# vLAR-group/unMORE

Hardware: AMD Instinct MI355X
Metric: images/sec (train fwd+bwd) ObjectnessNet ViT-B/16 384x384 (higher is better)
Workload: dtype bf16

## Files before the change

### include/umr.h

```cpp
#ifndef UMR_H
#define UMR_H
#include <stdint.h>

#ifdef __cplusplus
extern "C" {
#endif

typedef void* umr_stream_t;

enum umr_status { UMR_OK = 0, UMR_ERR_INVALID = -1, UMR_ERR_UNSUPPORTED = -2, UMR_ERR_HIP = -1000 };
enum umr_dtype { UMR_F32 = 0, UMR_BF16 = 1, UMR_BF16X3 = 2 };

int umr_version(void);
const char* umr_last_error_string(void);

enum umr_f32_mode { UMR_F32_EXACT = 0, UMR_F32_X3 = 1, UMR_F32_X3_FAST = 2 };
int umr_set_f32_mode(int mode);
int umr_get_f32_mode(void);

int umr_set_cu_budget(int cus);
int umr_get_cu_budget(void);

int umr_set_debug_option(const char* name, const char* value);
int umr_get_debug_option(const char* name, int* value, int* is_set);
// ... 40 lines not shown
int umr_unsplit3(const void* src, float* dst, int64_t rows, int K, int64_t ld_src, int64_t ld_dst, umr_stream_t stream);
int umr_split3_rows(const float* src, void* dst, int64_t rows, int K, int64_t ld_src, int64_t ld_dst, int rows_in, int rows_out,
                    int row_off, umr_stream_t stream);
int umr_gemm_nt_rowreduce_ok(const umr_gemm_desc* d);

typedef struct umr_gemm_tn_desc {
    const void* dY;
    const void* X;
    float* dW;
    float* dbias;
    void* workspace;
    int64_t workspace_bytes;
    int64_t lddy, ldx, lddw;
    int32_t M, N, K;
    int32_t dtype;
    int32_t accumulate;
    int32_t conv, nb, H, W, Cin, Ho, Wo;
    int32_t dy_rows_in, dy_rows_out, dy_row_off;
    int32_t x_rows_in, x_rows_out, x_row_off;
} umr_gemm_tn_desc;

int64_t umr_gemm_tn_workspace(const umr_gemm_tn_desc* d);
int umr_gemm_tn(const umr_gemm_tn_desc* d, umr_stream_t stream);

int umr_layernorm_fwd(const void* x, const float* gamma, const float* beta, void* y, float* mean, float* rstd,
                      int M, int D, float eps, int dtype, umr_stream_t stream);
int64_t umr_layernorm_bwd_workspace(int M, int D);
int umr_layernorm_bwd(const void* dy, const void* x, const float* gamma, const float* mean, const float* rstd,
                      const void* dres, void* dx, float* dgamma, float* dbeta, int accumulate, void* workspace,
                      int64_t workspace_bytes, int M, int D, int dtype, umr_stream_t stream);
int umr_layernorm_bwd_rows(const void* dy, const void* x, const float* gamma, const float* mean, const float* rstd,
                           const void* dres, void* dx, void* workspace, int64_t workspace_bytes, int M, int D, int dtype,
                           umr_stream_t stream);
int umr_layernorm_bwd_params(const void* workspace, int64_t workspace_bytes, float* dgamma, float* dbeta, int accumulate,
                             int M, int D, umr_stream_t stream);

int64_t umr_attention_bwd_workspace(int B, int N, int heads);
int umr_attention_fwd(const void* qkv, void* out, float* lse, int B, int N, int heads, int head_dim, int dtype,
                      umr_stream_t stream);
int umr_attention_bwd(const void* qkv, const void* out, const void* dout, const float* lse, float* dsum_ws, void* dqkv,
                      int B, int N, int heads, int head_dim, int dtype, umr_stream_t stream);

int umr_patchify(const float* images, void* out, int B, int H, int W, int patch, int ldk, int dtype, umr_stream_t stream);
int umr_bilinear_fwd(const void* x, void* y, int B, int Hi, int Wi, int Ho, int Wo, int C, int align_corners, int dtype, umr_stream_t stream);
int umr_bilinear_bwd(const void* dy, void* dx, int B, int Hi, int Wi, int Ho, int Wo, int C, int align_corners, int dtype, umr_stream_t stream);
#define UMR_BILINEAR_RELU 1
// ... 189 lines not shown
```

### unmore_amd/_lib.py

```python
import ctypes
import os
import subprocess

_HERE = os.path.dirname(os.path.abspath(__file__))
LIB_PATH = os.environ.get("UMR_LIB") or os.path.join(_HERE, "lib", "libumr.so")
CSRC = os.path.join(_HERE, "csrc")

F32, BF16, BF16X3 = 0, 1, 2
EPI_BIAS, EPI_ADD_AUX, EPI_MASK_RELU, EPI_MASK_DGELU, EPI_ADD_AUX2, EPI_OUT_F32, EPI_ROWBIAS, EPI_OUT_X3 = 1, 2, 4, 8, 16, 32, 64, 128
EPI_AUX_X3, EPI_AUX2_X3, EPI_C2_X3 = 256, 512, 1024
ACT_NONE, ACT_RELU, ACT_GELU, ACT_TANH = 0, 1, 2, 3
ACT_SIGMOID = 5
F32_EXACT, F32_X3, F32_X3_FAST = 0, 1, 2

_vp, _i32, _i64 = ctypes.c_void_p, ctypes.c_int32, ctypes.c_int64


class GemmDesc(ctypes.Structure):
    _fields_ = [("A", _vp), ("B", _vp), ("C", _vp), ("C2", _vp), ("bias", _vp), ("aux", _vp),
                ("aux2", _vp), ("rowbias", _vp),
                ("lda", _i64), ("ldb", _i64), ("ldc", _i64), ("ldc2", _i64), ("ldaux", _i64), ("ldaux2", _i64),
                ("M", _i32), ("N", _i32), ("K", _i32), ("dtype", _i32),
                ("flags", _i32), ("act", _i32), ("c2_mode", _i32), ("rows_per_batch", _i32),
                ("conv", _i32), ("nb", _i32), ("H", _i32), ("W", _i32), ("Cin", _i32), ("Ho", _i32), ("Wo", _i32),
                ("a_rows_in", _i32), ("a_rows_out", _i32), ("a_row_off", _i32),
                ("c_rows_in", _i32), ("c_rows_out", _i32), ("c_row_off", _i32), ("aux_mod", _i32),
                ("red_w", _vp), ("red_out", _vp), ("red_c", _i32), ("no_store", _i32)]


class GemmTnDesc(ctypes.Structure):
    _fields_ = [("dY", _vp), ("X", _vp), ("dW", _vp), ("dbias", _vp), ("workspace", _vp),
                ("workspace_bytes", _i64), ("lddy", _i64), ("ldx", _i64), ("lddw", _i64),
                ("M", _i32), ("N", _i32), ("K", _i32), ("dtype", _i32), ("accumulate", _i32),
                ("conv", _i32), ("nb", _i32), ("H", _i32), ("W", _i32), ("Cin", _i32), ("Ho", _i32), ("Wo", _i32),
                ("dy_rows_in", _i32), ("dy_rows_out", _i32), ("dy_row_off", _i32),
                ("x_rows_in", _i32), ("x_rows_out", _i32), ("x_row_off", _i32)]


class AdamPackEntry(ctypes.Structure):
    _fields_ = [("p", _vp), ("g", _vp), ("m", _vp), ("v", _vp), ("dst_lin", _vp), ("dst_t", _vp), ("n", _i64), ("N", _i32), ("K", _i32),
                ("blk_start", _i64)]


class BnBwdDesc(ctypes.Structure):
    _fields_ = [("dy", _vp), ("dpool", _vp), ("y", _vp), ("z", _vp * 2), ("mean", _vp * 2), ("rstd", _vp * 2), ("gamma", _vp * 2),
                ("dgamma", _vp * 2), ("dbeta", _vp * 2), ("dz", _vp * 2), ("g_out", _vp), ("workspace", _vp), ("workspace_bytes", _i64),
                ("rows_per_batch", _i64), ("pool_scale", ctypes.c_float), ("M", _i32), ("C", _i32), ("nbranch", _i32), ("dtype", _i32)]


class RaggedSrc(ctypes.Structure):
    _fields_ = [("f32", _vp), ("u8", _vp), ("H", _i32), ("W", _i32)]


class CpPair(ctypes.Structure):
    _fields_ = [("l_image", _vp), ("l_masks", _vp), ("l_boxes", _vp), ("u_image", _vp), ("u_masks", _vp), ("out_image", _vp), ("out_masks", _vp),
                ("word_off", _i64), ("inter_off", _i64), ("row_off", _i64), ("choice_off", _i64),
                ("Hl", _i32), ("Wl", _i32), ("Nl", _i32), ("Hu", _i32), ("Wu", _i32), ("Nu", _i32), ("nc", _i32), ("h_new", _i32), ("w_new", _i32),
                ("h_shift", _i32), ("w_shift", _i32), ("rh", ctypes.c_float), ("rw", ctypes.c_float), ("sx", ctypes.c_float), ("sy", ctypes.c_float),
                ("reserved", _i32)]
# ... 27 lines not shown
    "umr_label_synthesis_workspace": [_i32, _i32, _i32],
    "umr_label_synthesis": [_vp, _vp, _vp, _vp, _vp, _vp, _i64, _i32, _i32, _i32, _i32, _vp],
    "umr_label_synthesis_cropped": [_vp, _vp, _vp, _vp, _vp, _vp, _vp, _i64, _i32, _i32, _i32, _i32, _vp],
    "umr_crop_resize_batch": [_vp, _vp, _vp, _i32, _i32, _i32, _i32, _i32, _i32, _i32, _vp],
    "umr_distance_transform_workspace": [_i32, _i32, _i32],
    "umr_distance_transform": [_vp, _vp, _vp, _i64, _i32, _i32, _i32, _i32, _vp],
    "umr_bg_square_workspace": [_i32, _i64],
    "umr_bg_square": [_vp, _vp, _vp, _i64, _i32, _i32, _i64, _vp],
    "umr_crop_resize_ragged": [_vp, _vp, _vp, _vp, _vp, _i32, _i32, _i32, _i32, _vp],
    "umr_im2col_nchw": [_vp, _vp, _i32, _i32, _i32, _i32, _i32, _i32, _i32, _i32, _i32, _i32, _vp],
    "umr_maxpool3x3s2": [_vp, _vp, _i32, _i32, _i32, _i32, _i32, _vp],
    "umr_bn_fold": [_vp, _vp, _vp, _vp, _vp, _f32, _vp, _vp, _i32, _i32, _i32, _i32, _vp],
    "umr_bn_train_workspace": [_i32, _i32],
    "umr_bn_train_stats": [_vp, _vp, _vp, _vp, _vp, _vp, _vp, _i64, _i32, _i32, _f32, _f32, _i32, _vp],
    "umr_bn_train_apply": [_vp, _vp, _vp, _vp, _vp, _vp, _vp, _vp, _vp, _vp, _vp, _vp, _i32, _i32, _i32, _i32, _vp],
    "umr_bn_train_bwd_reduce": [_vp, _vp],
    "umr_bn_train_bwd_apply": [_vp, _vp],
    "umr_maxpool3x3s2_bwd": [_vp, _vp, _vp, _i32, _i32, _i32, _i32, _i32, _vp],
    "umr_stuff2_add": [_vp, _vp, _i32, _i32, _i32, _i32, _i32, _vp],
    "umr_bce_sigmoid": [_vp, _vp, _vp, _vp, _i32, _vp],
    "umr_head_out_finish": [_vp, _i32, _vp, _vp, _i64, _i32, _i32, _i32, _vp],
    "umr_gemm_tn": [_vp, _vp],
    "umr_gemm_tn_workspace": [_vp],
    "umr_layernorm_fwd": [_vp, _vp, _vp, _vp, _vp, _vp, _i32, _i32, _f32, _i32, _vp],
    "umr_layernorm_bwd_workspace": [_i32, _i32],
    "umr_layernorm_bwd": [_vp, _vp, _vp, _vp, _vp, _vp, _vp, _vp, _vp, _i32, _vp, _i64, _i32, _i32, _i32, _vp],
    "umr_layernorm_bwd_rows": [_vp, _vp, _vp, _vp, _vp, _vp, _vp, _vp, _i64, _i32, _i32, _i32, _vp],
    "umr_layernorm_bwd_params": [_vp, _i64, _vp, _vp, _i32, _i32, _i32, _vp],
    "umr_attention_fwd": [_vp, _vp, _vp, _i32, _i32, _i32, _i32, _i32, _vp],
    "umr_attention_bwd": [_vp, _vp, _vp, _vp, _vp, _vp, _i32, _i32, _i32, _i32, _i32, _vp],
    "umr_attention_bwd_workspace": [_i32, _i32, _i32],
    "umr_patchify": [_vp, _vp, _i32, _i32, _i32, _i32, _i32, _i32, _vp],
    "umr_bilinear_fwd": [_vp, _vp, _i32, _i32, _i32, _i32, _i32, _i32, _i32, _i32, _vp],
    "umr_bilinear_bwd": [_vp, _vp, _i32, _i32, _i32, _i32, _i32, _i32, _i32, _i32, _vp],
    "umr_bilinear_fwd_ex": [_vp, _i64, _vp, _i64, _i32, _i32, _i32, _i32, _i32, _i32, _i32, _i32, _i32, _vp],
    "umr_bilinear_bwd_ex": [_vp, _i64, _vp, _i64, _i32, _i32, _i32, _i32, _i32, _i32, _i32, _i32, _vp],
    "umr_pixel_shuffle": [_vp, _vp, _i32, _i32, _i32, _i32, _i32, _i32, _i32, _vp],
    "umr_zero_stuff2": [_vp, _vp, _i32, _i32, _i32, _i32, _i32, _i32, _i32, _vp],
    "umr_permute4": [_vp, _vp, _vp, _vp, _i64, _i32, _i32, _i32, _vp],
    "umr_segsum": [_vp, _vp, _i32, _i32, _i64, _i64, _i32, _i32, _i32, _i32, _vp],
    "umr_fill_cls": [_vp, _vp, _vp, _i32, _i64, _i32, _i32, _vp],
    "umr_cast": [_vp, _vp, _i64, _f32, _i32, _i32, _vp],
    "umr_scale_by_device_scalar": [_vp, _vp, _vp, _i64, _vp],
    "umr_head_out_fwd": [_vp, _vp, _vp, _vp, _i64, _i32, _i32, _i32, _i32, _i32, _vp],
    "umr_head_out_bwd_workspace": [_i64, _i32],
    "umr_head_out_bwd": [_vp, _vp, _vp, _vp, _vp, _vp, _vp, _vp, _i64, _i64, _i32, _i32, _i32, _i32, _i32, _i32, _vp],
# ... 86 lines not shown
```

### unmore_amd/csrc/gemm_tn.hip

```cpp
#include "umr_common.h"
#include <type_traits>
#include <stdlib.h>

namespace {

constexpr int TN_BN = 128, TN_BK = 128;
constexpr int TN_LDS = 65536;

template <typename T> struct TnTr;
template <> struct TnTr<bf16_t> { static constexpr int ROWS = 64, ROWB = 256, RPI = 4; };
template <> struct TnTr<float> { static constexpr int ROWS = 32, ROWB = 512, RPI = 2; };

__device__ __forceinline__ int tn_swz(int r) { return ((r & 3) << 2) | ((r >> 2) & 3); }

__device__ __forceinline__ void tn_split3(const float (&x)[8], bf16x8& h, bf16x8& m, bf16x8& l) {
#pragma unroll
    for (int e = 0; e < 8; ++e) {
        const bf16_t hh = (bf16_t)x[e];
        const float r = x[e] - (float)hh;
        const bf16_t mm = (bf16_t)r;
        h[e] = hh; m[e] = mm; l[e] = (bf16_t)(r - (float)mm);
    }
}

template <typename T, int CONV, bool X3 = false>
__global__ __launch_bounds__(256, 2) void gemm_tn_kernel(const umr_gemm_tn_desc p, int tiles_k, int rows_per_split,
                                                         float* slab, float* bslab) {
    extern __shared__ __attribute__((aligned(16))) char smem[];
    constexpr int ROWS = TnTr<T>::ROWS, ROWB = TnTr<T>::ROWB, RPI = TnTr<T>::RPI;
    constexpr int EPC = 16 / sizeof(T);
    constexpr int TILE = ROWS * ROWB;
    constexpr int STAGE = 2 * TILE;
    constexpr int CPR = ROWB / 16;
    const int tid = threadIdx.x, lane = tid & 63;
    const int w = __builtin_amdgcn_readfirstlane(tid >> 6);
    const int tile = blockIdx.x, split = blockIdx.y;
    const int tn = tile / tiles_k, tk = tile - tn * tiles_k;
    const int n0 = tn * TN_BN, k0 = tk * TN_BK;
    const int m_begin = split * rows_per_split;
    const int m_end = min(p.M, m_begin + rows_per_split);
    const bool do_bias = (p.dbias != nullptr) && (tk == 0);

    constexpr unsigned OOB = 0x80000000u;
    constexpr int SZ = (int)sizeof(T);
    const int lrow = lane / CPR, lchk = lane % CPR;
    const int stride = (CONV == 2) ? 2 : 1;
    int rr[4], gch[4], k_tap[4], k_ci[4], tky[4], tkx[4];
    unsigned y_vo[4], x_vo[4];
    bool k_ok[4];
#pragma unroll
    for (int i = 0; i < 4; ++i) {
        const int r = (w * 4 + i) * RPI + lrow;
        rr[i] = r;
        gch[i] = (sizeof(T) == 2) ? (lchk ^ tn_swz(r)) : lchk;
        const bool n_ok = (n0 + gch[i] * EPC) < p.N;
        y_vo[i] = n_ok ? (unsigned)(((int64_t)r * p.lddy) * SZ + gch[i] * 16) : OOB;
        const int kc = k0 + gch[i] * EPC;
        k_ok[i] = kc < p.K;
        k_tap[i] = 0;
// ... 250 lines not shown
                }
            }
        }
    }

    float* out = slab + (int64_t)split * p.N * p.K;
#pragma unroll
    for (int nt = 0; nt < 4; ++nt) {
        const int n = n0 + wn * 64 + nt * 16 + li;
        if (n >= p.N) continue;
#pragma unroll
        for (int kt = 0; kt < 4; ++kt) {
            const int k = k0 + wk * 64 + kt * 16 + g * 4;
            if (k >= p.K) continue;
            float* o = out + (int64_t)n * p.K + k;
            if (k + 3 < p.K && (p.K & 3) == 0) *(f32x4*)o = acc[nt][kt];
            else { for (int e = 0; e < 4; ++e) if (k + e < p.K) o[e] = acc[nt][kt][e]; }
        }
        if (do_bias && wk == 0 && g == 0) bslab[(int64_t)split * p.N + n] = accb[nt][0];
    }
}

template <int VEC>
__global__ void tn_reduce_kernel(const float* __restrict__ slab, float* __restrict__ dW, int64_t lddw, int N, int K,
                                 int splits, int accumulate, const float* __restrict__ bslab, float* __restrict__ dbias, int bias_parts) {
    const int64_t total = (int64_t)N * K;
    const int64_t nvec = total / VEC;
    for (int64_t iv = (int64_t)blockIdx.x * blockDim.x + threadIdx.x; iv < nvec; iv += (int64_t)gridDim.x * blockDim.x) {
        const int64_t i = iv * VEC;
        const int n = (int)(i / K), k = (int)(i - (int64_t)n * K);
        float* o = dW + (int64_t)n * lddw + k;
        if (VEC == 4) {
            f32x4 s0 = {0.f, 0.f, 0.f, 0.f}, s1 = s0, s2 = s0, s3 = s0;
            const float* q = slab + i;
            int sp = 0;
            for (; sp + 4 <= splits; sp += 4) {
                s0 += *(const f32x4*)(q + (int64_t)(sp + 0) * total);
                s1 += *(const f32x4*)(q + (int64_t)(sp + 1) * total);
                s2 += *(const f32x4*)(q + (int64_t)(sp + 2) * total);
                s3 += *(const f32x4*)(q + (int64_t)(sp + 3) * total);
            }
            for (; sp < splits; ++sp) s0 += *(const f32x4*)(q + (int64_t)sp * total);
            f32x4 r = (s0 + s1) + (s2 + s3);
            if (accumulate) r += *(const f32x4*)o;
            *(f32x4*)o = r;
        } else {
            float sacc = 0.f;
            for (int sp = 0; sp < splits; ++sp) sacc += slab[(int64_t)sp * total + i];
            *o = accumulate ? (*o + sacc) : sacc;
        }
    }
    if (dbias != nullptr) {
        for (int n = blockIdx.x * blockDim.x + threadIdx.x; n < N; n += gridDim.x * blockDim.x) {
            float b0 = 0.f, b1 = 0.f, b2 = 0.f, b3 = 0.f;
            int sp = 0;
            for (; sp + 4 <= bias_parts; sp += 4) {
                b0 += bslab[(int64_t)(sp + 0) * N + n];
                b1 += bslab[(int64_t)(sp + 1) * N + n];
                b2 += bslab[(int64_t)(sp + 2) * N + n];
                b3 += bslab[(int64_t)(sp + 3) * N + n];
            }
            for (; sp < bias_parts; ++sp) b0 += bslab[(int64_t)sp * N + n];
            const float sacc = (b0 + b1) + (b2 + b3);
            dbias[n] = accumulate ? (dbias[n] + sacc) : sacc;
        }
    }
}

struct TnPlan { int tiles_n, tiles_k, splits, rows_per_split; int64_t ws; bool big; };

}
bool umr_tn256_eligible(const umr_gemm_tn_desc* d, bool force);
void umr_tn256_plan(const umr_gemm_tn_desc* d, int* splits, int* rows_per_split);
int umr_launch_gemm_tn256(const umr_gemm_tn_desc* d, int splits, int rows_per_split, float* slab, float* bslab, hipStream_t s);
namespace {

static int tn_tile_override() {
    return umr_opt_or(UMR_OPT_GEMM_TILE, 0);
}

TnPlan tn_plan(const umr_gemm_tn_desc* d) {
    TnPlan pl;
    pl.big = tn_tile_override() != 128 && umr_tn256_eligible(d, tn_tile_override() == 256);
    if (pl.big) {
        pl.tiles_n = (d->N + 255) / 256;
        pl.tiles_k = (d->K + 255) / 256;
        umr_tn256_plan(d, &pl.splits, &pl.rows_per_split);
        pl.ws = ((int64_t)pl.splits * d->N * d->K + (int64_t)pl.splits * pl.tiles_k * d->N) * 4;
        return pl;
// ... 6 lines not shown
    int64_t max_by_rows = ((int64_t)d->M + rows * 8 - 1) / (rows * 8);
    if (d->M <= 4096) {
        want = (256 + tiles / 2) / tiles;
        max_by_rows = ((int64_t)d->M + rows * 4 - 1) / (rows * 4);
    }
    if (want > max_by_rows) want = max_by_rows;
    if (want < 1) want = 1;
    if (want > 4096) want = 4096;
    int64_t rps = ((int64_t)d->M + want - 1) / want;
    rps = (rps + rows - 1) / rows * rows;
    pl.rows_per_split = (int)rps;
    pl.splits = (int)(((int64_t)d->M + rps - 1) / rps);
    pl.ws = ((int64_t)pl.splits * d->N * d->K + (int64_t)pl.splits * d->N) * 4;
    return pl;
}

}

extern "C" int64_t umr_gemm_tn_workspace(const umr_gemm_tn_desc* d) {
    if (!d || d->M <= 0 || d->N <= 0 || d->K <= 0) return 0;
    return tn_plan(d).ws;
}

extern "C" int umr_gemm_tn(const umr_gemm_tn_desc* d, umr_stream_t stream) {
    UMR_CHECK_ARG(d != nullptr, "gemm_tn: null descriptor");
    UMR_CHECK_ARG(d->dY && d->X && d->dW && d->workspace, "gemm_tn: null operand");
    UMR_CHECK_ARG(d->M > 0 && d->N > 0 && d->K > 0, "gemm_tn: empty problem");
    UMR_CHECK_ARG(d->dtype == UMR_F32 || d->dtype == UMR_BF16 || d->dtype == UMR_BF16X3, "gemm_tn: dtype");
    const int epc = d->dtype == UMR_F32 ? 4 : 8;
    if (d->dtype == UMR_BF16X3) {
        if (d->dy_rows_in > 0 || d->x_rows_in > 0 || d->conv == 2)
            return umr_set_error(UMR_ERR_UNSUPPORTED, "gemm_tn (BF16X3): no row remaps, no stride-2 conv");
        UMR_CHECK_ARG(d->lddy >= 3 * (int64_t)d->N && (d->conv != 0 || d->ldx >= 3 * (int64_t)d->K), "gemm_tn (BF16X3): rows hold three planes (lddy >= 3N, ldx >= 3K)");
    }
    UMR_CHECK_ARG(d->N % epc == 0 && d->lddy % epc == 0, "gemm_tn: N/lddy must be multiples of 16 bytes");
    UMR_CHECK_ARG(d->conv >= 0 && d->conv <= 2, "gemm_tn: conv mode");
    if (d->conv == 0) {
        UMR_CHECK_ARG(d->K % epc == 0 && d->ldx % epc == 0, "gemm_tn: K/ldx must be multiples of 16 bytes");
    } else {
        UMR_CHECK_ARG(d->Cin % epc == 0 && d->K == 9 * d->Cin, "gemm_tn: conv needs Cin % 16B == 0 and K == 9*Cin");
        UMR_CHECK_ARG((int64_t)d->nb * d->Ho * d->Wo == d->M, "gemm_tn: conv M != nb*Ho*Wo");
        const int s = d->conv == 2 ? 2 : 1;
        UMR_CHECK_ARG(d->Ho == (d->H - 1) / s + 1 && d->Wo == (d->W - 1) / s + 1, "gemm_tn: conv output size");
    }
    {
        const int rows = d->dtype == UMR_F32 ? 32 : 64;
        const int64_t sz = d->dtype == UMR_F32 ? 4 : 2;
        const bool remap = d->dy_rows_in > 0 || (d->conv == 0 && d->x_rows_in > 0);
        const bool conv_general = d->conv != 0 && !(d->conv == 1 && d->Wo % rows == 0);
        (void)conv_general;
        if (remap) {
            const int64_t ymax = d->dy_rows_in > 0 ? ((int64_t)d->M / d->dy_rows_in + 1) * d->dy_rows_out : d->M;
            const int64_t xmax = d->x_rows_in > 0 ? ((int64_t)d->M / d->x_rows_in + 1) * d->x_rows_out : d->M;
            if (ymax * d->lddy * sz >= (1ll << 31) || (d->conv == 0 && xmax * d->ldx * sz >= (1ll << 31)))
                return umr_set_error(UMR_ERR_UNSUPPORTED, "gemm_tn: row-remapped operands must be < 2 GiB");
        }
    }
    const TnPlan pl = tn_plan(d);
    UMR_CHECK_ARG(d->workspace_bytes >= pl.ws, "gemm_tn: workspace too small");
    hipStream_t s = (hipStream_t)stream;
    float* slab = (float*)d->workspace;
    float* bslab = slab + (int64_t)pl.splits * d->N * d->K;
    const bool direct = !pl.big && pl.splits == 1 && !d->accumulate && d->lddw == d->K &&
                        ((uintptr_t)d->dW & 15) == 0;
    if (direct) { slab = d->dW; bslab = d->dbias; }
    if (pl.big) {
        const int st = umr_launch_gemm_tn256(d, pl.splits, pl.rows_per_split, slab, bslab, s);
        if (st != UMR_OK) return st;
    } else {
    dim3 g((unsigned)(pl.tiles_n * pl.tiles_k), (unsigned)pl.splits), b(256);
#define LAUNCH(T, CV) hipLaunchKernelGGL((gemm_tn_kernel<T, CV>), g, b, TN_LDS, s, *d, pl.tiles_k, pl.rows_per_split, slab, bslab)
#define LAUNCH_X3(CV) hipLaunchKernelGGL((gemm_tn_kernel<float, CV, true>), g, b, TN_LDS, s, *d, pl.tiles_k, pl.rows_per_split, slab, bslab)
    const int f32_x3 = umr_f32_mode_now() != UMR_F32_EXACT;
    if (d->dtype == UMR_BF16) {
        if (d->conv == 0) LAUNCH(bf16_t, 0); else if (d->conv == 1) LAUNCH(bf16_t, 1); else LAUNCH(bf16_t, 2);
    } else if (f32_x3) {
        if (d->conv == 0) LAUNCH_X3(0); else if (d->conv == 1) LAUNCH_X3(1); else LAUNCH_X3(2);
    } else {
        if (d->conv == 0) LAUNCH(float, 0); else if (d->conv == 1) LAUNCH(float, 1); else LAUNCH(float, 2);
    }
#undef LAUNCH_X3
#undef LAUNCH
    UMR_LAUNCH_CHECK();
    }
    if (direct) return UMR_OK;
    const int64_t total = (int64_t)d->N * d->K;
    const bool v4 = (d->K % 4 == 0) && (d->lddw % 4 == 0) && (((uintptr_t)d->dW & 15) == 0);
    int rb = (int)((total / (v4 ? 4 : 1) + 255) / 256);
    if (rb > 8192) rb = 8192;
    if (rb < 1) rb = 1;
    if (v4)
        hipLaunchKernelGGL(tn_reduce_kernel<4>, dim3(rb), dim3(256), 0, s, slab, d->dW, d->lddw, d->N, d->K, pl.splits,
                           d->accumulate, bslab, d->dbias, pl.big ? pl.splits * pl.tiles_k : pl.splits);
    else
        hipLaunchKernelGGL(tn_reduce_kernel<1>, dim3(rb), dim3(256), 0, s, slab, d->dW, d->lddw, d->N, d->K, pl.splits,
                           d->accumulate, bslab, d->dbias, pl.big ? pl.splits * pl.tiles_k : pl.splits);
    UMR_LAUNCH_CHECK();
    return UMR_OK;
}
```

### unmore_amd/csrc/gemm_tn256.hip

```cpp
#include "umr_common.h"
#include <type_traits>
#include <stdlib.h>

namespace {

constexpr int TSUB = 64 * 256;
constexpr int TBUF = 4 * TSUB;
constexpr int TLDS = 2 * TBUF;

__device__ __forceinline__ int tn_swz2(int r) { return ((r & 3) << 2) | ((r >> 2) & 3); }

template <int CONV, bool PH2, int WF, bool X3 = false>
__global__ __launch_bounds__(512, 2) void gemm_tn256_kernel(const umr_gemm_tn_desc p, int tiles_k, int ntiles, int rows_per_split,
                                                            float* slab, float* bslab, int mapmode, int npairs_arg = 1) {
    extern __shared__ __attribute__((aligned(16))) char smem[];
    constexpr int SZ = 2;
    const int npairs = X3 ? npairs_arg : 1;
    const int xpix = X3 ? 3 * p.Cin : p.Cin;
    constexpr unsigned OOB = 0x80000000u;
    const int tid = threadIdx.x, lane = tid & 63;
    const int w = __builtin_amdgcn_readfirstlane(tid >> 6);
    int bid = blockIdx.x;
    {
        const int nwg = gridDim.x, xcd = bid & 7, q_ = nwg >> 3, r_ = nwg & 7;
// ... 293 lines not shown
        for (int kt = 0; kt < 4; ++kt) {
            const int k = (mapmode & 1) ? k0 + (kt >> 1) * 128 + wk * 32 + (kt & 1) * 16 + g * 4 : k0 + wk * 64 + kt * 16 + g * 4;
            if (k >= p.K) continue;
            float* o = out + (int64_t)n * p.K + k;
            if (k + 3 < p.K && (p.K & 3) == 0) *(f32x4*)o = acc[nt][kt];
            else { for (int e = 0; e < 4; ++e) if (k + e < p.K) o[e] = acc[nt][kt][e]; }
        }
        if (do_bias && wk == 0) {
            float s_ = bsum[nt];
            s_ += __shfl_xor(s_, 16, 64);
            s_ += __shfl_xor(s_, 32, 64);
            if (g == 0) bslab[((int64_t)split * tiles_k + tk) * p.N + n] = s_;
        }
    }
}

}

bool umr_tn256_eligible(const umr_gemm_tn_desc* d, bool force) {
    if (d->dtype != UMR_BF16 && d->dtype != UMR_BF16X3) return false;
    if (d->dy_rows_in > 0 || d->x_rows_in > 0) return false;
    if (d->conv == 2) return false;
    if (d->dtype == UMR_BF16X3) return true;
    if (d->conv == 1 && d->Wo < 64) return false;
    if (force) return true;
    if (d->N < 192 || d->K < 192) return false;
    const int64_t tiles = (int64_t)((d->N + 255) / 256) * ((d->K + 255) / 256);
    return (int64_t)d->M >= 256 * 64 * 16 / (tiles < 1 ? 1 : tiles) && d->M >= 64 * 64;
}

void umr_tn256_plan(const umr_gemm_tn_desc* d, int* splits, int* rows_per_split) {
    const int64_t tiles = (int64_t)((d->N + 255) / 256) * ((d->K + 255) / 256);
    const int x3 = d->dtype == UMR_BF16X3 ? 6 : 1;
    int64_t rounds = (int64_t)d->M * tiles * x3 / (256ll * 4096);
    if (rounds < 1) rounds = 1;
    if (rounds > 4) rounds = 4;
    int64_t want = rounds * 256 / tiles;
    if (want < 1) want = 1;
    const int64_t min_stages = x3 == 6 ? 2 : 16;
    const int64_t max_by_rows = ((int64_t)d->M + 64 * min_stages - 1) / (64 * min_stages);
    if (want > max_by_rows) want = max_by_rows;
    int64_t rps = ((int64_t)d->M + want - 1) / want;
    rps = (rps + 63) / 64 * 64;
    {
        const int64_t cpix = (int64_t)d->Cin * (d->dtype == UMR_BF16X3 ? 3 : 1);
        const int64_t rowb = 2 * (int64_t)(d->conv ? (cpix > d->lddy ? cpix : d->lddy) : (d->ldx > d->lddy ? d->ldx : d->lddy));
        const int64_t halo = d->conv ? (2 * (int64_t)d->W + 4) * cpix * 2 : 0;
        int64_t cap = ((1ll << 31) - halo - 65536) / rowb / 64 * 64;
// ... 6 lines not shown

int umr_launch_gemm_tn256(const umr_gemm_tn_desc* d, int splits, int rows_per_split, float* slab, float* bslab, hipStream_t s) {
    const int tiles_n = (d->N + 255) / 256, tiles_k = (d->K + 255) / 256;
    dim3 g((unsigned)(tiles_n * tiles_k * splits)), b(512);
    constexpr int mapmode = 3;
#define LT(CV, WFV)                                                                                                    \
    do {                                                                                                               \
        UMR_SET_MAX_LDS_ONCE((gemm_tn256_kernel<CV, true, WFV>), TLDS);                                                \
        hipLaunchKernelGGL((gemm_tn256_kernel<CV, true, WFV>), g, b, TLDS, s, *d, tiles_k, tiles_n * tiles_k, rows_per_split, slab, bslab, mapmode, 1); \
    } while (0)
#define LTX(CV, WFV)                                                                                                   \
    do {                                                                                                               \
        UMR_SET_MAX_LDS_ONCE((gemm_tn256_kernel<CV, true, WFV, true>), TLDS);                                          \
        hipLaunchKernelGGL((gemm_tn256_kernel<CV, true, WFV, true>), g, b, TLDS, s, *d, tiles_k, tiles_n * tiles_k, rows_per_split, slab, bslab, mapmode, npairs); \
    } while (0)
    if (d->dtype == UMR_BF16X3) {
        const int npairs = umr_f32_mode_now() == UMR_F32_X3_FAST ? 3 : 6;
        if (d->conv == 0) LTX(0, 0);
        else if (d->Wo % 64 == 0) LTX(1, 1);
        else if (d->Wo >= 64) LTX(1, 0);
        else LTX(1, 2);
    } else if (d->conv == 0) LT(0, 0);
    else if (d->Wo % 64 == 0) LT(1, 1);
    else LT(1, 0);
#undef LTX
#undef LT
    UMR_LAUNCH_CHECK();
    return UMR_OK;
}
```

### unmore_amd/engine.py

```python
import os

import torch

from . import _lib as L
from . import graphs
from . import ops
from .engine_x3 import X3Numerics, _drop_f, _f
from .packs import (ParamGroup, PackCache, _ACT, _pack_conv3, _pack_conv3_dgrad, _pack_convT, _pack_convT_dgrad, _pack_linear,
                    _pack_linear_t, _rep_bias, _unpack_conv3_grad)

CONFIGS = {
    "dpt_large": dict(D=1024, depth=24, heads=16, patch=16, pos_grid=24, hooks=[5, 11, 17, 23], features=[256, 512, 1024, 1024]),
    "dpt_base": dict(D=768, depth=12, heads=12, patch=16, pos_grid=24, hooks=[2, 5, 8, 11], features=[96, 192, 384, 768]),
    "dpt_small": dict(D=384, depth=12, heads=6, patch=16, pos_grid=24, hooks=[2, 5, 8, 11], features=[48, 96, 192, 384]),
    "dpt_large14": dict(D=1024, depth=24, heads=16, patch=14, pos_grid=37, hooks=[5, 11, 17, 23], features=[256, 512, 1024, 1024]),
    "dpt_tiny": dict(D=128, depth=4, heads=2, patch=16, pos_grid=24, hooks=[0, 1, 2, 3], features=[32, 64, 128, 128]),
}

_FUSE_HEAD_OUT = True
_COMMUTE_RESIZE = True


_WGRAD_STREAM = os.environ.get("UMR_WGRAD_STREAM", "auto")
_side_streams = {}


class WgradStream:

    def __init__(self, dev, on):
        self.on = bool(on)
        self.staged = graphs.staged() if self.on else None
        if self.on and self.staged is None:
            self.main = torch.cuda.current_stream(dev)
            key = (dev.index, self.main.cuda_stream)
            if key not in _side_streams:
                if len(_side_streams) > 16:
                    _side_streams.clear()
                _side_streams[key] = torch.cuda.Stream(device=dev)
            self.side = _side_streams[key]

    def run(self, fn, *used):
        if not self.on:
            return fn()
        if self.staged is not None:
            return self.staged.defer(fn, used)
        self.side.wait_stream(self.main)
        graphs.note_fork(self.main, self.side)
# ... 18 lines not shown
        if _WGRAD_STREAM in ("0", "1"):
            return _WGRAD_STREAM == "1"
        return pixels <= graphs.AUTO_MAX_PIXELS


class PlainNumerics:

    def __init__(self, e, P):
        self.e, self.P = e, P

    def val(self, t):
        return t

    def to_dt(self, t):
        return t if self.e.dt == torch.float32 else ops.cast(t, self.e.dt)

    def mm(self, A, wname, kind, bias=None, *, conv=0, act=L.ACT_NONE, want="f", mask=None, dgelu=None, aux=None, aux2=None,
           rowbias=None, rows_per_batch=0, c2_mode=0, c2_want="f", out=None, c_remap=None, aux_mod=0):
        a_t = mask if mask is not None else (dgelu if dgelu is not None else aux)
        return ops.gemm_nt(A, self.e._w(self.P, wname, kind), bias, out=out, aux=a_t, aux2=aux2, rowbias=rowbias,
                           rows_per_batch=rows_per_batch, act=act, mask_relu=mask is not None, mask_dgelu=dgelu is not None,
                           c2_mode=c2_mode, conv=conv, c_remap=c_remap, aux_mod=aux_mod)

    def wgrad(self, dY, X, dW, dbias=None, *, conv=0, wg=None, then=None):
        def launch():
            r = ops.gemm_tn(dY, X, dW=dW, dbias=dbias, conv=conv)
            if then is not None:
                then(r)
            return r
        return launch() if wg is None else wg.run(launch, dY, X)

    def layernorm(self, x, gamma, beta):
        return ops.layernorm_fwd(x, gamma, beta)

    def readout(self, tok, wname, bias, save, B, g, Nt, D):
        P, dt = self.P, self.e.dt
        w_full = self.e.cache.get((wname, "lin", dt), P[wname], lambda: _pack_linear(P[wname], dt))
        rb = ops.gemm_nt(tok, w_full[:, D:], bias, M=B, lda=Nt * D, out_f32=True)
        if save:
            r, rpre = ops.gemm_nt(tok, w_full[:, :D], None, rowbias=rb, rows_per_batch=g, act=L.ACT_GELU, c2_mode=2, M=B * g,
                                  a_remap=(g, Nt, 1))
        else:
            r, rpre = ops.gemm_nt(tok, w_full[:, :D], None, rowbias=rb, rows_per_batch=g, act=L.ACT_GELU, M=B * g,
                                  a_remap=(g, Nt, 1)), None
        return dict(r=r, rpre=rpre)

    def readout_wgrad(self, d_rpre, rs, tok, dW, B, g, Nt):
        ops.gemm_tn(d_rpre, tok, dW=dW, x_remap=(g, Nt, 1), M=B * g)

    def hook_grad(self, d_rpre, sB, wname, dx, B, g, Nt, D):
        dt = self.e.dt
        w = self.P[wname].detach()
# ... 483 lines not shown
                              aux=(hs["h1"] if relu else None), mask_relu=relu)
            del dh2
            hs["h1"] = None
            ops.bilinear_bwd(dh1.view(B, H, W, c1), ph, pw, True, out=dlow[:, c0:c0 + c1].unflatten(0, (nb, ph, pw)))
            del dh1
            wgrad_lin(f"{name}.{idx[0]}.weight", dlow[:, c0:c0 + c1], pl, f"{name}.{idx[0]}.bias")
            bcat[:, c0:c0 + c1].copy_(self._w(P, f"{name}.{idx[0]}.weight", "lin_t"))
            c0 += c1
        dpath = ops.gemm_nt(dlow, bcat, None).view(nb, ph, pw, C)
        S["path"] = None
        S["feat"] = None
        return dpath

    def backward(self, P, S, d_center, d_sdf, G, stage_cb=None, join_at_stages=False):
        cfg = self.cfg
        nx = S["numerics"](self, P)
        mm, val = nx.mm, nx.val
        B, H, W, gh, gw = S["B"], S["H"], S["W"], S["gh"], S["gw"]
        D, heads, p = cfg["D"], cfg["heads"], cfg["patch"]
        g, Nt = gh * gw, gh * gw + 1
        dev = d_center.device
        wg = WgradStream(dev, WgradStream.wanted(B * H * W))
        ln_via = wg.run if wg.staged is not None else None

        def cb(name):
            if join_at_stages:
                wg.join()
            if stage_cb is not None:
                stage_cb(name, wg)
            wg.stage_end()

        def wgrad_lin(name, dy, x, bias_name=None):
            nx.wgrad(dy, x, G[name].view(G[name].shape[0], -1), (G[bias_name] if bias_name else None), wg=wg)

        def wgrad_c3(name, dy, x_nhwc, bias_name=None, conv=1):
            co = G[name].shape[0]
            nx.wgrad(dy.view(-1, co), x_nhwc, None, (G[bias_name] if bias_name else None), conv=conv, wg=wg,
                     then=lambda dwp: _unpack_conv3_grad(dwp, G[name]))

        dpath = nx.heads_backward(S, d_center, d_sdf, G, wgrad_lin, wgrad_c3, lambda: cb("heads"))

        sc = "backbone.scratch."
        d_rn = {}
        for k in (1, 2, 3, 4):
            r_ = sc + f"refinenet{k}."
            fs = S["fus"][k]
            hh, ww = fs["in_hw"]
            nb, Hp, Wp = dpath.shape[0], dpath.shape[1], dpath.shape[2]
            shp = (nb, hh, ww, 256)
            if "u" in fs:
                dul = val(ops.bilinear_bwd(_f(dpath), hh, ww, True)).view(nb * hh * ww, 256)
                wgrad_lin(r_ + "out_conv.weight", dul, fs["u"].view(nb * hh * ww, 256), r_ + "out_conv.bias")
                du = mm(dul, r_ + "out_conv.weight", "lin_t", None).view(*shp)
                del dul
            else:
                dp2 = dpath.view(nb * Hp * Wp, 256)
                wgrad_lin(r_ + "out_conv.weight", dp2, fs["up"].view(nb * Hp * Wp, 256), r_ + "out_conv.bias")
                dup = _f(mm(dp2, r_ + "out_conv.weight", "lin_t", None))
                du = val(ops.bilinear_bwd(dup.view(nb, Hp, Wp, 256), hh, ww, True))
                del dup
            wgrad_c3(r_ + "resConfUnit2.conv2.weight", du, fs["t2"], r_ + "resConfUnit2.conv2.bias")
# ... 118 lines not shown
```

### unmore_amd/ops.py

```python
import collections
import ctypes

import torch

from . import _lib as L
from . import graphs

_DT = {torch.float32: L.F32, torch.bfloat16: L.BF16}


_cur_dev = torch._C._cuda_getDevice
_raw_stream = torch._C._cuda_getCurrentRawStream


def _stream_id(device_index=None):
    return _raw_stream(_cur_dev() if device_index is None else device_index)


def _stream():
    return ctypes.c_void_p(_raw_stream(_cur_dev()))


def _p(t):
    return ctypes.c_void_p(t.data_ptr()) if t is not None else None
# ... 296 lines not shown
        d.aux, d.ldaux = _p(t2), ld
        keep.append(t2)
    if aux2 is not None:
        t2, ld, pl = _x3_operand(aux2, N)
        flags |= L.EPI_ADD_AUX2 | (L.EPI_AUX2_X3 if pl else 0)
        d.aux2, d.ldaux2 = _p(t2), ld
        keep.append(t2)
    if c2_mode:
        assert red_w is None and c_remap is None
        out2 = torch.empty((M_, 3 * N if c2_planes else N), dtype=torch.bfloat16 if c2_planes else torch.float32, device=Ap.device)
        flags |= L.EPI_C2_X3 if c2_planes else 0
        d.C2, d.ldc2, d.c2_mode = _p(out2), out2.stride(0), c2_mode
    d.aux_mod = aux_mod
    d.A, d.B, d.C, d.bias = _p(Ap), _p(Bp), _p(out), _p(bias)
    d.ldb = Bp.stride(0)
    d.M, d.N, d.K, d.dtype = M_, N, K, L.BF16X3
    d.flags, d.act, d.conv = flags, act, conv
    L.check(_timed_call(d), "umr_gemm_nt")
    if red_w is not None:
        return partials
    return (out, out2) if c2_mode else out


def gemm_tn(dY, X, *, dW=None, dbias=None, accumulate=False, conv=0, M=None, dy_remap=None, x_remap=None, lddy=None, ldx=None, x3=False):
    _need_gpu(dY, X)
    dt = L.BF16X3 if x3 else _DT[X.dtype]
    assert dY.dtype == X.dtype and (not x3 or X.dtype == torch.bfloat16)
    pl = 3 if x3 else 1
    d = L.GemmTnDesc()
    dY2 = dY.reshape(-1, dY.shape[-1]) if dY.is_contiguous() else dY
    N = dY2.shape[-1] // pl
    M = dY2.shape[0] if M is None else M
    if conv:
        nb, H, W, Cin = X.shape
        Cin //= pl
        assert X.is_contiguous()
        s = 2 if conv == 2 else 1
        Ho, Wo = (H - 1) // s + 1, (W - 1) // s + 1
        assert M == nb * Ho * Wo
        K = 9 * Cin
        d.nb, d.H, d.W, d.Cin, d.Ho, d.Wo = nb, H, W, Cin, Ho, Wo
        d.ldx = Cin * pl
    else:
        X2 = X.reshape(-1, X.shape[-1]) if X.is_contiguous() else X
        K = X2.shape[-1] // pl
        d.ldx = X2.stride(0) if ldx is None else ldx
    if dW is None:
        dW = torch.empty((N, K), dtype=torch.float32, device=X.device)
        assert not accumulate
    assert dW.dtype == torch.float32 and dW.stride(-1) == 1
    if dbias is not None:
        assert dbias.dtype == torch.float32 and dbias.numel() == N
    d.dY, d.X, d.dW, d.dbias = _p(dY2), _p(X), _p(dW), _p(dbias)
    d.lddy, d.lddw = (dY2.stride(0) if lddy is None else lddy), (dW.stride(0) if dW.dim() == 2 else K)
    if dy_remap is not None:
        d.dy_rows_in, d.dy_rows_out, d.dy_row_off = dy_remap
    if x_remap is not None:
        d.x_rows_in, d.x_rows_out, d.x_row_off = x_remap
    d.M, d.N, d.K, d.dtype, d.accumulate, d.conv = M, N, K, dt, int(accumulate), conv
    need = L.lib().umr_gemm_tn_workspace(ctypes.byref(d))
    ws = _workspace(need, X.device)
    d.workspace, d.workspace_bytes = _p(ws), ws.numel()
    L.check(L.lib().umr_gemm_tn(ctypes.byref(d), _stream()), "umr_gemm_tn")
    return dW


def layernorm_fwd(x, gamma, beta, eps=1e-6, planes=False):
    _need_gpu(x)
    D = x.shape[-1]
    x2 = x.reshape(-1, D)
    M = x2.shape[0]
    mean = torch.empty(M, dtype=torch.float32, device=x.device)
    rstd = torch.empty(M, dtype=torch.float32, device=x.device)
    if planes:
        assert x.dtype == torch.float32
        y = torch.empty((M, 3 * D), dtype=torch.bfloat16, device=x.device)
        L.check(L.lib().umr_layernorm_fwd(_p(x2), _p(gamma), _p(beta), _p(y), _p(mean), _p(rstd), M, D, eps, L.BF16X3, _stream()),
                "umr_layernorm_fwd")
        return y, mean, rstd
    y = torch.empty_like(x2)
    L.check(L.lib().umr_layernorm_fwd(_p(x2), _p(gamma), _p(beta), _p(y), _p(mean), _p(rstd), M, D, eps, _DT[x.dtype], _stream()),
            "umr_layernorm_fwd")
    return y.view(x.shape), mean, rstd


def layernorm_bwd(dy, x, gamma, mean, rstd, dgamma, dbeta, dres=None, accumulate=False, params_via=None):
# ... 553 lines not shown
```

Measured before the change: 356.7.

## Defer and batch split-K weight-gradient reductions across head wgrads

Adds a deferred mode to the TN wgrad GEMM. The split-K slab reduction is recorded instead of launched, and the recorded reductions are run together in one batched kernel at each stage boundary in the heads backward, cutting kernel-launch count. The wgrad kernel grid is also flattened to 1D with an XCD-aware block remap, and the 256-tile path is now taken under force even for small-Wo conv. The cost is a separate workspace allocation per deferred GEMM instead of the shared one, so more memory is held.

```diff
diff --git a/include/umr.h b/include/umr.h
--- a/include/umr.h
+++ b/include/umr.h
@@ -86,6 +86,16 @@
 
 int64_t umr_gemm_tn_workspace(const umr_gemm_tn_desc* d);
 int umr_gemm_tn(const umr_gemm_tn_desc* d, umr_stream_t stream);
+
+#define UMR_TN_REDUCE_MAX 8
+typedef struct umr_tn_reduce_entry {
+    const float* slab; float* dW; const float* bslab; float* dbias;
+    int64_t lddw;
+    int32_t N, K, splits, accumulate, bias_parts, vec4;
+    int32_t blocks, blk_start;
+} umr_tn_reduce_entry;
+int umr_gemm_tn_deferred(const umr_gemm_tn_desc* d, umr_tn_reduce_entry* entry, umr_stream_t stream);
+int umr_tn_reduce_batched(const umr_tn_reduce_entry* entries, int n, umr_stream_t stream);
 
 int umr_layernorm_fwd(const void* x, const float* gamma, const float* beta, void* y, float* mean, float* rstd,
                       int M, int D, float eps, int dtype, umr_stream_t stream);
diff --git a/unmore_amd/_lib.py b/unmore_amd/_lib.py
--- a/unmore_amd/_lib.py
+++ b/unmore_amd/_lib.py
@@ -35,6 +35,15 @@
                 ("conv", _i32), ("nb", _i32), ("H", _i32), ("W", _i32), ("Cin", _i32), ("Ho", _i32), ("Wo", _i32),
                 ("dy_rows_in", _i32), ("dy_rows_out", _i32), ("dy_row_off", _i32),
                 ("x_rows_in", _i32), ("x_rows_out", _i32), ("x_row_off", _i32)]
+
+
+TN_REDUCE_MAX = 8
+
+
+class TnReduceEntry(ctypes.Structure):
+    _fields_ = [("slab", _vp), ("dW", _vp), ("bslab", _vp), ("dbias", _vp), ("lddw", _i64),
+                ("N", _i32), ("K", _i32), ("splits", _i32), ("accumulate", _i32), ("bias_parts", _i32), ("vec4", _i32),
+                ("blocks", _i32), ("blk_start", _i32)]
 
 
 class AdamPackEntry(ctypes.Structure):
@@ -108,6 +117,8 @@
     "umr_head_out_finish": [_vp, _i32, _vp, _vp, _i64, _i32, _i32, _i32, _vp],
     "umr_gemm_tn": [_vp, _vp],
     "umr_gemm_tn_workspace": [_vp],
+    "umr_gemm_tn_deferred": [_vp, _vp, _vp],
+    "umr_tn_reduce_batched": [_vp, _i32, _vp],
     "umr_layernorm_fwd": [_vp, _vp, _vp, _vp, _vp, _vp, _i32, _i32, _f32, _i32, _vp],
     "umr_layernorm_bwd_workspace": [_i32, _i32],
     "umr_layernorm_bwd": [_vp, _vp, _vp, _vp, _vp, _vp, _vp, _vp, _vp, _i32, _vp, _i64, _i32, _i32, _i32, _vp],
diff --git a/unmore_amd/csrc/gemm_tn.hip b/unmore_amd/csrc/gemm_tn.hip
--- a/unmore_amd/csrc/gemm_tn.hip
+++ b/unmore_amd/csrc/gemm_tn.hip
@@ -24,7 +24,7 @@
 }
 
 template <typename T, int CONV, bool X3 = false>
-__global__ __launch_bounds__(256, 2) void gemm_tn_kernel(const umr_gemm_tn_desc p, int tiles_k, int rows_per_split,
+__global__ __launch_bounds__(256, 2) void gemm_tn_kernel(const umr_gemm_tn_desc p, int tiles_k, int ntiles, int rows_per_split,
                                                          float* slab, float* bslab) {
     extern __shared__ __attribute__((aligned(16))) char smem[];
     constexpr int ROWS = TnTr<T>::ROWS, ROWB = TnTr<T>::ROWB, RPI = TnTr<T>::RPI;
@@ -34,7 +34,13 @@
     constexpr int CPR = ROWB / 16;
     const int tid = threadIdx.x, lane = tid & 63;
     const int w = __builtin_amdgcn_readfirstlane(tid >> 6);
-    const int tile = blockIdx.x, split = blockIdx.y;
+    int bid = blockIdx.x;
+    {
+        const int nwg = gridDim.x, xcd = bid & 7, q_ = nwg >> 3, r_ = nwg & 7;
+        const int base = (xcd < r_) ? xcd * (q_ + 1) : r_ * (q_ + 1) + (xcd - r_) * q_;
+        bid = base + (bid >> 3);
+    }
+    const int split = bid / ntiles, tile = bid - split * ntiles;
     const int tn = tile / tiles_k, tk = tile - tn * tiles_k;
     const int n0 = tn * TN_BN, k0 = tk * TN_BK;
     const int m_begin = split * rows_per_split;
@@ -331,11 +337,12 @@
 }
 
 template <int VEC>
-__global__ void tn_reduce_kernel(const float* __restrict__ slab, float* __restrict__ dW, int64_t lddw, int N, int K,
-                                 int splits, int accumulate, const float* __restrict__ bslab, float* __restrict__ dbias, int bias_parts) {
+__device__ __forceinline__ void tn_reduce_body(const float* __restrict__ slab, float* __restrict__ dW, int64_t lddw, int N, int K,
+                                               int splits, int accumulate, const float* __restrict__ bslab, float* __restrict__ dbias,
+                                               int bias_parts, int bid, int nblk) {
     const int64_t total = (int64_t)N * K;
     const int64_t nvec = total / VEC;
-    for (int64_t iv = (int64_t)blockIdx.x * blockDim.x + threadIdx.x; iv < nvec; iv += (int64_t)gridDim.x * blockDim.x) {
+    for (int64_t iv = (int64_t)bid * blockDim.x + threadIdx.x; iv < nvec; iv += (int64_t)nblk * blockDim.x) {
         const int64_t i = iv * VEC;
         const int n = (int)(i / K), k = (int)(i - (int64_t)n * K);
         float* o = dW + (int64_t)n * lddw + k;
@@ -360,7 +367,7 @@
         }
     }
     if (dbias != nullptr) {
-        for (int n = blockIdx.x * blockDim.x + threadIdx.x; n < N; n += gridDim.x * blockDim.x) {
+        for (int n = bid * blockDim.x + threadIdx.x; n < N; n += nblk * blockDim.x) {
             float b0 = 0.f, b1 = 0.f, b2 = 0.f, b3 = 0.f;
             int sp = 0;
             for (; sp + 4 <= bias_parts; sp += 4) {
@@ -374,6 +381,23 @@
             dbias[n] = accumulate ? (dbias[n] + sacc) : sacc;
         }
     }
+}
+
+template <int VEC>
+__global__ void tn_reduce_kernel(const float* __restrict__ slab, float* __restrict__ dW, int64_t lddw, int N, int K,
+                                 int splits, int accumulate, const float* __restrict__ bslab, float* __restrict__ dbias, int bias_parts) {
+    tn_reduce_body<VEC>(slab, dW, lddw, N, K, splits, accumulate, bslab, dbias, bias_parts, (int)blockIdx.x, (int)gridDim.x);
+}
+
+struct TnReduceTable { umr_tn_reduce_entry e[UMR_TN_REDUCE_MAX]; int n; };
+__global__ __launch_bounds__(256) void tn_reduce_batched_kernel(const TnReduceTable t) {
+    const int b = (int)blockIdx.x;
+    int i = 0;
+    while (i + 1 < t.n && b >= t.e[i + 1].blk_start) ++i;
+    const umr_tn_reduce_entry& e = t.e[i];
+    const int bid = b - e.blk_start;
+    if (e.vec4) tn_reduce_body<4>(e.slab, e.dW, e.lddw, e.N, e.K, e.splits, e.accumulate, e.bslab, e.dbias, e.bias_parts, bid, e.blocks);
+    else tn_reduce_body<1>(e.slab, e.dW, e.lddw, e.N, e.K, e.splits, e.accumulate, e.bslab, e.dbias, e.bias_parts, bid, e.blocks);
 }
 
 struct TnPlan { int tiles_n, tiles_k, splits, rows_per_split; int64_t ws; bool big; };
@@ -426,7 +450,35 @@
     return tn_plan(d).ws;
 }
 
-extern "C" int umr_gemm_tn(const umr_gemm_tn_desc* d, umr_stream_t stream) {
+static int tn_gemm_impl(const umr_gemm_tn_desc* d, umr_tn_reduce_entry* defer, umr_stream_t stream);
+
+extern "C" int umr_gemm_tn(const umr_gemm_tn_desc* d, umr_stream_t stream) { return tn_gemm_impl(d, nullptr, stream); }
+
+extern "C" int umr_gemm_tn_deferred(const umr_gemm_tn_desc* d, umr_tn_reduce_entry* entry, umr_stream_t stream) {
+    UMR_CHECK_ARG(entry != nullptr, "gemm_tn_deferred: null entry");
+    return tn_gemm_impl(d, entry, stream);
+}
+
+extern "C" int umr_tn_reduce_batched(const umr_tn_reduce_entry* entries, int n, umr_stream_t stream) {
+    UMR_CHECK_ARG(entries != nullptr && n > 0 && n <= UMR_TN_REDUCE_MAX, "tn_reduce_batched: 1 .. UMR_TN_REDUCE_MAX entries");
+    TnReduceTable t;
+    int64_t blk = 0;
+    for (int i = 0; i < n; ++i) {
+        t.e[i] = entries[i];
+        UMR_CHECK_ARG(t.e[i].slab && t.e[i].dW && t.e[i].splits > 0 && t.e[i].blocks > 0 && t.e[i].N > 0 && t.e[i].K > 0,
+                      "tn_reduce_batched: entry not filled by umr_gemm_tn_deferred");
+        t.e[i].blk_start = (int32_t)blk;
+        blk += t.e[i].blocks;
+    }
+    for (int i = n; i < UMR_TN_REDUCE_MAX; ++i) t.e[i] = umr_tn_reduce_entry{};
+    t.n = n;
+    hipLaunchKernelGGL(tn_reduce_batched_kernel, dim3((unsigned)blk), dim3(256), 0, (hipStream_t)stream, t);
+    UMR_LAUNCH_CHECK();
+    return UMR_OK;
+}
+
+static int tn_gemm_impl(const umr_gemm_tn_desc* d, umr_tn_reduce_entry* defer, umr_stream_t stream) {
+    if (defer) defer->splits = 0;
     UMR_CHECK_ARG(d != nullptr, "gemm_tn: null descriptor");
     UMR_CHECK_ARG(d->dY && d->X && d->dW && d->workspace, "gemm_tn: null operand");
     UMR_CHECK_ARG(d->M > 0 && d->N > 0 && d->K > 0, "gemm_tn: empty problem");
@@ -472,9 +524,11 @@
         const int st = umr_launch_gemm_tn256(d, pl.splits, pl.rows_per_split, slab, bslab, s);
         if (st != UMR_OK) return st;
     } else {
-    dim3 g((unsigned)(pl.tiles_n * pl.tiles_k), (unsigned)pl.splits), b(256);
-#define LAUNCH(T, CV) hipLaunchKernelGGL((gemm_tn_kernel<T, CV>), g, b, TN_LDS, s, *d, pl.tiles_k, pl.rows_per_split, slab, bslab)
-#define LAUNCH_X3(CV) hipLaunchKernelGGL((gemm_tn_kernel<float, CV, true>), g, b, TN_LDS, s, *d, pl.tiles_k, pl.rows_per_split, slab, bslab)
+    const int ntiles = pl.tiles_n * pl.tiles_k;
+    UMR_CHECK_ARG((int64_t)ntiles * pl.splits < (1ll << 31), "gemm_tn: too many workgroups");
+    dim3 g((unsigned)(ntiles * pl.splits)), b(256);
+#define LAUNCH(T, CV) hipLaunchKernelGGL((gemm_tn_kernel<T, CV>), g, b, TN_LDS, s, *d, pl.tiles_k, ntiles, pl.rows_per_split, slab, bslab)
+#define LAUNCH_X3(CV) hipLaunchKernelGGL((gemm_tn_kernel<float, CV, true>), g, b, TN_LDS, s, *d, pl.tiles_k, ntiles, pl.rows_per_split, slab, bslab)
     const int f32_x3 = umr_f32_mode_now() != UMR_F32_EXACT;
     if (d->dtype == UMR_BF16) {
         if (d->conv == 0) LAUNCH(bf16_t, 0); else if (d->conv == 1) LAUNCH(bf16_t, 1); else LAUNCH(bf16_t, 2);
@@ -493,6 +547,12 @@
     int rb = (int)((total / (v4 ? 4 : 1) + 255) / 256);
     if (rb > 8192) rb = 8192;
     if (rb < 1) rb = 1;
+    if (defer) {
+        defer->slab = slab; defer->dW = d->dW; defer->bslab = bslab; defer->dbias = d->dbias;
+        defer->lddw = d->lddw; defer->N = d->N; defer->K = d->K; defer->splits = pl.splits; defer->accumulate = d->accumulate;
+        defer->bias_parts = pl.big ? pl.splits * pl.tiles_k : pl.splits; defer->vec4 = v4 ? 1 : 0; defer->blocks = rb; defer->blk_start = 0;
+        return UMR_OK;
+    }
     if (v4)
         hipLaunchKernelGGL(tn_reduce_kernel<4>, dim3(rb), dim3(256), 0, s, slab, d->dW, d->lddw, d->N, d->K, pl.splits,
                            d->accumulate, bslab, d->dbias, pl.big ? pl.splits * pl.tiles_k : pl.splits);
diff --git a/unmore_amd/csrc/gemm_tn256.hip b/unmore_amd/csrc/gemm_tn256.hip
--- a/unmore_amd/csrc/gemm_tn256.hip
+++ b/unmore_amd/csrc/gemm_tn256.hip
@@ -339,8 +339,8 @@
     if (d->dy_rows_in > 0 || d->x_rows_in > 0) return false;
     if (d->conv == 2) return false;
     if (d->dtype == UMR_BF16X3) return true;
+    if (force) return true;
     if (d->conv == 1 && d->Wo < 64) return false;
-    if (force) return true;
     if (d->N < 192 || d->K < 192) return false;
     const int64_t tiles = (int64_t)((d->N + 255) / 256) * ((d->K + 255) / 256);
     return (int64_t)d->M >= 256 * 64 * 16 / (tiles < 1 ? 1 : tiles) && d->M >= 64 * 64;
@@ -393,7 +393,8 @@
         else LTX(1, 2);
     } else if (d->conv == 0) LT(0, 0);
     else if (d->Wo % 64 == 0) LT(1, 1);
-    else LT(1, 0);
+    else if (d->Wo >= 64) LT(1, 0);
+    else LT(1, 2);
 #undef LTX
 #undef LT
     UMR_LAUNCH_CHECK();
diff --git a/unmore_amd/engine.py b/unmore_amd/engine.py
--- a/unmore_amd/engine.py
+++ b/unmore_amd/engine.py
@@ -23,6 +23,7 @@
 
 _WGRAD_STREAM = os.environ.get("UMR_WGRAD_STREAM", "auto")
 _side_streams = {}
+_DEFER_TN_REDUCE = os.environ.get("UMR_TN_DEFER_REDUCE", "1") != "0"
 
 
 class WgradStream:
@@ -87,12 +88,9 @@
                            rows_per_batch=rows_per_batch, act=act, mask_relu=mask is not None, mask_dgelu=dgelu is not None,
                            c2_mode=c2_mode, conv=conv, c_remap=c_remap, aux_mod=aux_mod)
 
-    def wgrad(self, dY, X, dW, dbias=None, *, conv=0, wg=None, then=None):
+    def wgrad(self, dY, X, dW, dbias=None, *, conv=0, wg=None, then=None, defer=None):
         def launch():
-            r = ops.gemm_tn(dY, X, dW=dW, dbias=dbias, conv=conv)
-            if then is not None:
-                then(r)
-            return r
+            return ops.gemm_tn(dY, X, dW=dW, dbias=dbias, conv=conv, defer=defer, then=then)
         return launch() if wg is None else wg.run(launch, dY, X)
 
     def layernorm(self, x, gamma, beta):
@@ -622,8 +620,12 @@
         dev = d_center.device
         wg = WgradStream(dev, WgradStream.wanted(B * H * W))
         ln_via = wg.run if wg.staged is not None else None
+        batch = ops.TnReduceBatch() if (_DEFER_TN_REDUCE and not wg.on and isinstance(nx, PlainNumerics)) else None
+        dfr = dict(defer=batch) if batch is not None else {}
 
         def cb(name):
+            if batch is not None:
+                batch.flush()
             if join_at_stages:
                 wg.join()
             if stage_cb is not None:
@@ -631,12 +633,12 @@
             wg.stage_end()
 
         def wgrad_lin(name, dy, x, bias_name=None):
-            nx.wgrad(dy, x, G[name].view(G[name].shape[0], -1), (G[bias_name] if bias_name else None), wg=wg)
+            nx.wgrad(dy, x, G[name].view(G[name].shape[0], -1), (G[bias_name] if bias_name else None), wg=wg, **dfr)
 
         def wgrad_c3(name, dy, x_nhwc, bias_name=None, conv=1):
             co = G[name].shape[0]
             nx.wgrad(dy.view(-1, co), x_nhwc, None, (G[bias_name] if bias_name else None), conv=conv, wg=wg,
-                     then=lambda dwp: _unpack_conv3_grad(dwp, G[name]))
+                     then=lambda dwp: _unpack_conv3_grad(dwp, G[name]), **dfr)
 
         dpath = nx.heads_backward(S, d_center, d_sdf, G, wgrad_lin, wgrad_c3, lambda: cb("heads"))
 
diff --git a/unmore_amd/ops.py b/unmore_amd/ops.py
--- a/unmore_amd/ops.py
+++ b/unmore_amd/ops.py
@@ -342,7 +342,31 @@
     return (out, out2) if c2_mode else out
 
 
-def gemm_tn(dY, X, *, dW=None, dbias=None, accumulate=False, conv=0, M=None, dy_remap=None, x_remap=None, lddy=None, ldx=None, x3=False):
+class TnReduceBatch:
+    MAX_SLAB_BYTES = 192 << 20
+    launches = 0
+
+    def __init__(self):
+        self.entries, self.keep, self.thens = [], [], []
+
+    def __len__(self):
+        return len(self.entries)
+
+    def flush(self):
+        n = len(self.entries)
+        for i in range(0, n, L.TN_REDUCE_MAX):
+            chunk = self.entries[i:i + L.TN_REDUCE_MAX]
+            arr = (L.TnReduceEntry * len(chunk))(*chunk)
+            L.check(L.lib().umr_tn_reduce_batched(arr, len(chunk), _stream()), "umr_tn_reduce_batched")
+            TnReduceBatch.launches += 1
+        thens, self.thens = self.thens, []
+        self.entries, self.keep = [], []
+        for fn, dW in thens:
+            fn(dW)
+
+
+def gemm_tn(dY, X, *, dW=None, dbias=None, accumulate=False, conv=0, M=None, dy_remap=None, x_remap=None, lddy=None, ldx=None, x3=False,
+            defer=None, then=None):
     _need_gpu(dY, X)
     dt = L.BF16X3 if x3 else _DT[X.dtype]
     assert dY.dtype == X.dtype and (not x3 or X.dtype == torch.bfloat16)
@@ -379,9 +403,23 @@
         d.x_rows_in, d.x_rows_out, d.x_row_off = x_remap
     d.M, d.N, d.K, d.dtype, d.accumulate, d.conv = M, N, K, dt, int(accumulate), conv
     need = L.lib().umr_gemm_tn_workspace(ctypes.byref(d))
-    ws = _workspace(need, X.device)
-    d.workspace, d.workspace_bytes = _p(ws), ws.numel()
-    L.check(L.lib().umr_gemm_tn(ctypes.byref(d), _stream()), "umr_gemm_tn")
+    if defer is not None and need <= TnReduceBatch.MAX_SLAB_BYTES:
+        ws = torch.empty(max(int(need), 16), dtype=torch.uint8, device=X.device)
+        d.workspace, d.workspace_bytes = _p(ws), ws.numel()
+        e = L.TnReduceEntry()
+        L.check(L.lib().umr_gemm_tn_deferred(ctypes.byref(d), ctypes.byref(e), _stream()), "umr_gemm_tn_deferred")
+        if e.splits > 0:
+            defer.entries.append(e)
+            defer.keep.append((ws, dW, dbias))
+            if then is not None:
+                defer.thens.append((then, dW))
+            return dW
+    else:
+        ws = _workspace(need, X.device)
+        d.workspace, d.workspace_bytes = _p(ws), ws.numel()
+        L.check(L.lib().umr_gemm_tn(ctypes.byref(d), _stream()), "umr_gemm_tn")
+    if then is not None:
+        then(dW)
     return dW
 
 
```

New measurement: 356.0. About the same (-0.2%).
